# Linxyhaha/AtSpeed

Hardware: AMD Instinct MI355X
Metric: recommended items/sec (K=20 beams per user), mean accepted length alongside (higher is better)
Workload: dtype bf16; 1 GPU; Beauty V=32859, Llama-68M draft / Llama-7B(32L) target, K=20, DK=40, gamma=4, L=4, 256 user(s) per lock-step batch per GPU, position-set mask; users_per_gpu=1280, parallelism=user-shard x1

## Files before the change

### atspeed_amd/_lib.py

```python
from __future__ import annotations

import ctypes as C
import os
from typing import Optional

_HERE = os.path.dirname(os.path.abspath(__file__))
LIB_PATH = os.path.abspath(os.environ["ATSPEED_LIB"]) if os.environ.get("ATSPEED_LIB") else os.path.join(_HERE, "lib", "libatspeed_hip.so")

ATSPEED_F32, ATSPEED_BF16, ATSPEED_F16 = 0, 1, 2
WEIGHTS_ROW_MAJOR, WEIGHTS_PACKED = 0, 1
MAX_BEAMS, MAX_NEW_TOKENS, MAX_GAMMA = 64, 16, 8
LORA_MAX_RANK = 64
LORA_MAX_ADAPTERS = 16
ERR_INVALID, ERR_HIP, ERR_CAPACITY, ERR_CONSTRAINT, ERR_NO_DEVICE, ERR_FILTERED = -1, -2, -3, -4, -5, -6
EPI_STORE, EPI_F32, EPI_RESID, EPI_SWIGLU = 0, 1, 2, 3
MASK_BLOCK, MASK_ALLOW = 0, 1


class LlamaLayerWeights(C.Structure):
    _fields_ = [("input_norm", C.c_void_p), ("wqkv", C.c_void_p), ("wo", C.c_void_p),
                ("post_norm", C.c_void_p), ("wgu", C.c_void_p), ("wd", C.c_void_p)]


class LlamaConfig(C.Structure):
    _fields_ = [("vocab_size", C.c_int32), ("hidden", C.c_int32), ("n_layers", C.c_int32), ("n_heads", C.c_int32),
                ("ffn", C.c_int32), ("rope_theta", C.c_float), ("rms_eps", C.c_float), ("dtype", C.c_int32),
                ("max_slots", C.c_int32), ("max_tokens", C.c_int32), ("max_logit_rows", C.c_int32), ("weight_layout", C.c_int32)]


class LoraLayer(C.Structure):
    _fields_ = [("a_q", C.c_void_p), ("b_q", C.c_void_p), ("a_k", C.c_void_p), ("b_k", C.c_void_p), ("a_v", C.c_void_p), ("b_v", C.c_void_p)]


class LoraSlot(C.Structure):
    _fields_ = [("a_cat", C.c_void_p), ("b_q", C.c_void_p), ("b_k", C.c_void_p), ("b_v", C.c_void_p), ("r16", C.c_int32), ("scaling", C.c_float)]


class GenStats(C.Structure):
    _fields_ = [("n_run", C.c_int32), ("total_accept_steps", C.c_int32), ("accept_steps", C.c_int32 * MAX_NEW_TOKENS),
                ("n_valid", C.c_int32), ("n_target_forwards", C.c_int32), ("n_draft_forwards", C.c_int32),
                ("draft_ms", C.c_float), ("target_ms", C.c_float), ("verify_ms", C.c_float), ("total_ms", C.c_float),
                ("status", C.c_int32), ("n_target_passes", C.c_int32)]


class SessionCounters(C.Structure):
    _fields_ = [("rounds", C.c_int64), ("target_forwards", C.c_int64), ("draft_forwards", C.c_int64), ("lane_rounds", C.c_int64),
                ("users_admitted", C.c_int64), ("users_retired", C.c_int64), ("allocs_after_create", C.c_int64),
                ("arena_reserved", C.c_int32), ("arena_failed", C.c_int32), ("n_lanes", C.c_int32), ("lanes_occupied", C.c_int32),
                ("queued", C.c_int64), ("target_passes", C.c_int64)]


class SessionDone(C.Structure):
    _fields_ = [("ticket", C.c_int64), ("lane", C.c_int32), ("status", C.c_int32), ("rounds_queued", C.c_int64),
                ("rounds_in_lane", C.c_int64)]


class SessionUser(C.Structure):
    _fields_ = [("struct_size", C.c_size_t), ("prompt_ids_dev", C.c_void_p), ("prompt_len", C.c_int32), ("start_node", C.c_int32),
                ("seed", C.c_uint32), ("out_tokens_dev", C.c_void_p), ("out_scores_dev", C.c_void_p), ("stats_host", C.POINTER(GenStats)),
                ("masks", C.c_void_p), ("mask_user", C.c_int32), ("adapter", C.c_int32)]


_P, _I, _F, _SZ, _U32, _U64 = C.c_void_p, C.c_int32, C.c_float, C.c_size_t, C.c_uint32, C.c_uint64
_SEGS = [_I, _P, _P, _P, _P, _P, _P, _P, _P, _P]
SIGNATURES = {
    "atspeed_version": (C.c_char_p, []),
    "atspeed_last_error": (C.c_char_p, []),
    "atspeed_device_count": (C.c_int, []),
    "atspeed_fill_hash_normal": (C.c_int, [_P, _SZ, _U32, _F, _F, C.c_int, _U64, _P]),
    "atspeed_fsm_create": (C.c_int, [_P, _P, _P, _I, _I, _I, C.POINTER(_P)]),
    "atspeed_fsm_destroy": (None, [_P]),
    "atspeed_fsm_create_free": (C.c_int, [_I, C.POINTER(_P)]),
    "atspeed_fsm_set_id_filter": (C.c_int, [_P, _I, _I]),
    "atspeed_row_topk": (C.c_int, [_P, _I, _I, _I, _I, _P, _P]),
    "atspeed_beam_expand_prune_free": (C.c_int, [_P, _I, _P, _P, _I, _I, _I, _P, _P, _P, _P, _P, _P]),
    "atspeed_trie_flatten": (C.c_int, [_P, _P, _I, _P, _P, _P, C.POINTER(_I), C.POINTER(_I)]),
    "atspeed_llama_create": (C.c_int, [C.POINTER(LlamaConfig), _P, _P, _P, C.POINTER(LlamaLayerWeights), C.POINTER(_P)]),
    "atspeed_llama_destroy": (None, [_P]),
    "atspeed_llama_forward": (C.c_int, [_P, _P, _P, _P, _P, _I, _I, _I, _P, _P]),
    "atspeed_llama_forward_batch": (C.c_int, [_P, _I, _P, _P, _P, _P, _P, _P, _P, _P, _P]),
    "atspeed_llama_logits": (_P, [_P]),
    "atspeed_llama_read": (C.c_int, [_P, _I, _I, _P, _SZ, _P]),
    "atspeed_probe_mfma_bf16": (C.c_int, [_I, _P, C.c_size_t, _P, _P]),
    "atspeed_probe_hbm_read": (C.c_int, [_P, C.c_size_t, _I, _P, _P, _P]),
    "atspeed_llama_enable_fp8": (C.c_int, [_P, _P]),
    "atspeed_llama_fp8_counters": (C.c_int, [_P, _P, _P, _I]),
    "atspeed_llama_enable_fp4": (C.c_int, [_P, _P]),
    "atspeed_llama_fp4_counters": (C.c_int, [_P, _P, _P, _I]),
    "atspeed_quant_weights_mxfp4": (C.c_int, [_P, _I, _I, _I, _I, _P, _P, _P]),
    "atspeed_gemm_w4a8": (C.c_int, [_P, _P, _P, _P, _P, _I, _I, _I, _I, _I, _I, _I, _P, _SZ, _P]),
    "atspeed_llama_rope_fused_launches": (C.c_int64, [_P, _I]),
    "atspeed_llama_sk_arena_bytes": (C.c_int64, [_P]),
    "atspeed_llama_set_lora": (C.c_int, [_P, _I, _F, C.POINTER(LoraLayer), _P]),
    "atspeed_llama_clear_lora": (C.c_int, [_P]),
    "atspeed_llama_lora_launches": (C.c_int64, [_P, _I]),
# ... 184 lines not shown
```

### atspeed_amd/beamSD.py

```python
from __future__ import annotations

import ctypes as C
import time
import weakref
from types import SimpleNamespace
from typing import Dict, Optional

import numpy as np
import torch

from . import _lib
from .generation_trie import ConstraintFSM, SuffixTrieConstraint, WholeSentenceTrieConstraint, free_constraint
from .model import HipLlama


class Timer:

    def __init__(self, func="", sync_cuda=True, syn_device=0):
        self.func = func
        self.sync_cuda = sync_cuda
        self.syn_device = syn_device

    def _sync(self):
        if self.sync_cuda and torch.cuda.is_available():
# ... 364 lines not shown
    for i in range(n):
        o0, P = k * (int(off[i]) + i * L), int(off[i + 1] - off[i])
        res.append({"beam_sequence": out[o0: o0 + k * (P + L)].view(k, P + L), "beam_scores": scores[i]})
    return res


def _batch_call(entry, c: SimpleNamespace, k: int, max_new_tokens: int, *middle):
    n = len(c.prompts)
    ptrs, ints = C.c_void_p * n, C.c_int32 * n
    with torch.cuda.device(c.dev):
        ids32, toks, scores, keep = _batch_buffers(c.prompts, k, max_new_tokens, c.dev)
        stats = (_lib.GenStats * n)()
        try:
            _lib.check(entry(ptrs(*[d.handle for d in c.decs]), n, ptrs(*[t.data_ptr() for t in ids32]),
                             ints(*[int(p.numel()) for p in c.prompts]), c.dfsm.handle, ints(*[f.start for f in c.fsms]), *middle,
                             ptrs(*[t.data_ptr() for t in toks]), ptrs(*[t.data_ptr() for t in scores]), stats, _lib.stream_ptr(c.dev)))
        finally:
            if c.filter_owners:
                _clear_filters(c.decs)
    return (keep, toks, scores, k), stats


MAX_USERS_PER_CALL = 256


def _chunk_of(lists, i: int, n: int):
    return None if lists is None else lists[i:i + n]


def _chunked(call, inputs_list, mode):
    outs = []
    for i in range(0, len(inputs_list), MAX_USERS_PER_CALL):
        outs += call(inputs_list[i:i + MAX_USERS_PER_CALL], (mode[2] + i) if mode[0] else None, i)
    return outs


def _bssd_stats(st, k: int) -> Dict:
    n_run = int(st.n_run)
    total = int(st.total_accept_steps)
    return {
        "n_run": n_run,
        "total_accept_steps": total,
        "total_accept_tokens": total * k,
        "ave_accept_tokens": total * k / n_run if n_run else 0.0,
        "draft_time_cost": st.draft_ms * 1e-3,
        "target_time_cost": st.target_ms * 1e-3,
        "verify_time_cost": st.verify_ms * 1e-3,
        "device_time_cost": st.total_ms * 1e-3,
        "accept_steps": [int(st.accept_steps[i]) for i in range(min(n_run, _lib.MAX_NEW_TOKENS))],
        "n_valid": int(st.n_valid),
        "n_target_forwards": int(st.n_target_forwards),
        "n_draft_forwards": int(st.n_draft_forwards),
        "n_target_passes": int(st.n_target_passes),
    }


@Timer()
@torch.no_grad()
def BSSD(target_model, draft_model, inputs: Dict, gamma: int, max_new_tokens: int,
         logits_processor=None, prefix_allowed_tokens_fn=None, seed=None, trace_decisions: bool = False,
         exclude_items=None, allow_items=None, adapter=None) -> Dict:
    mode = _mode(seed, target_model, draft_model)
    filters = _filter_specs(1, exclude_items, allow_items, False, "BSSD")
    slots = _adapter_slots(target_model, adapter, 1, False, "BSSD")
    if _host_path(logits_processor, prefix_allowed_tokens_fn):
        _refuse_host_filters(filters, "BSSD")
        _refuse_host_adapters(slots, "BSSD")
        from .hostmask import bssd_host_mask
        return _host_call(bssd_host_mask, (target_model, draft_model), inputs, (int(gamma), int(max_new_tokens)), logits_processor,
                          prefix_allowed_tokens_fn, mode)
    k = int(target_model.generation_config.num_beams)
    dk = int(draft_model.generation_config.num_beams)
    c = _setup(target_model, draft_model, [inputs], prefix_allowed_tokens_fn, mode, "BSSD", trace_decisions, filters, adapters=slots)
    out, stats = _one_user_call(_lib.load().atspeed_bssd_generate, c, k, max_new_tokens, int(gamma), int(max_new_tokens), k, dk)
    out.update(_bssd_stats(stats, k))
    return out


beam_sd_generate = BSSD


class BSSDSession:

    def __init__(self, target_model, draft_model, lanes: int, gamma: int, max_new_tokens: int, prefix_allowed_tokens_fn=None,
                 max_prompt: Optional[int] = None, seed=None, logits_processor=None, trace_decisions: bool = False, _cached_decoders: bool = False):
        self.mode = _mode(seed, target_model, draft_model)
        if _host_path(logits_processor, prefix_allowed_tokens_fn):
            raise ValueError("BSSDSession runs on the device only: the mask must be able to compile() itself and there is no logits_processor")
        if trace_decisions:
            raise ValueError("BSSDSession keeps no decision trace: use BSSD / BSSD_batch with trace_decisions=True")
        if not 1 <= int(lanes) <= MAX_USERS_PER_CALL:
            raise ValueError(f"BSSDSession: lanes must be in 1 .. {MAX_USERS_PER_CALL}, not {lanes}")
        self.target, self.draft, self.fn = target_model, draft_model, prefix_allowed_tokens_fn
        self.n_lanes, self.gamma, self.max_new_tokens = int(lanes), int(gamma), int(max_new_tokens)
        self.k = int(target_model.generation_config.num_beams)
        self.dk = int(draft_model.generation_config.num_beams)
        self.max_prompt = int(max_prompt) if max_prompt is not None else min(target_model.max_tokens, 512)
        self.dev = target_model.device
        self._cached_decoders = _cached_decoders
        self._owner = self._decs = self._dfsm = self._fsm0 = None
        self._users: Dict[int, SimpleNamespace] = {}
        self._done_buf = (_lib.SessionDone * (2 * self.n_lanes))()
        self._submitted, self._closed = 0, False

    def _create(self, fsm: ConstraintFSM) -> None:
        lib = _lib.load()
# ... 271 lines not shown
```

### atspeed_amd/csrc/engine.hip

```cpp
#include <math.h>
#include <stdarg.h>
#include <string.h>

#include <algorithm>
#include <map>
#include <memory>
#include <mutex>
#include <vector>

#include "internal.h"
#include "session_queue.h"

static thread_local std::string g_last_error;

void atspeed_set_error(const char* fmt, ...) {
  char buf[1024];
  va_list ap;
  va_start(ap, fmt);
  vsnprintf(buf, sizeof(buf), fmt, ap);
  va_end(ap);
  g_last_error = buf;
}

extern "C" const char* atspeed_last_error(void) { return g_last_error.c_str(); }
std::atomic<long long> g_ats_lazy_allocs{0};
extern "C" const char* atspeed_version(void) { return "atspeed_hip 0.2 (gfx950)"; }

namespace {
constexpr int ATS_VERIFY_STAGED_TOKENS = 4096;
constexpr int ATS_VERIFY_STAGED_PASS_TOKENS = 1024;
constexpr int ATS_TAIL_ROWS_TOKENS = 512;
struct SwDef { const char* name; const char* env; int dflt; };
const SwDef kSwitches[ATS_N_SW] = {{"gemm_sk", "ATSPEED_GEMM_SK", 1},           {"gemm_sk_g", nullptr, 0},
                                   {"gemm_panel", "ATSPEED_GEMM_PANEL", 1},     {"gemm_force_mt", "ATSPEED_GEMM_FORCE_MT", 0},
                                   {"graphs", "ATSPEED_GRAPHS", 0},             {"fuse_qkv_rope", "ATSPEED_FUSE_QKV_ROPE", 1},
                                   {"gemm_kcut", "ATSPEED_GEMM_KCUT", 2},       {"fuse_qkv_reduce", "ATSPEED_FUSE_QKV_REDUCE", 1},
                                   {"verify_staged", "ATSPEED_VERIFY_STAGED", 1},
                                   {"verify_staged_tokens", "ATSPEED_VERIFY_STAGED_TOKENS", ATS_VERIFY_STAGED_TOKENS},
                                   {"verify_staged_pass_tokens", "ATSPEED_VERIFY_STAGED_PASS_TOKENS", ATS_VERIFY_STAGED_PASS_TOKENS},
                                   {"tail_rows_tokens", "ATSPEED_TAIL_ROWS_TOKENS", ATS_TAIL_ROWS_TOKENS},
                                   {"attn_short", "ATSPEED_ATTN_SHORT", 1}};
std::atomic<int> g_switch[ATS_N_SW];
std::once_flag g_switch_once;
void switches_init() {
  std::call_once(g_switch_once, [] {
    for (int i = 0; i < ATS_N_SW; ++i) {
      const char* v = kSwitches[i].env ? getenv(kSwitches[i].env) : nullptr;
      g_switch[i].store(v ? atoi(v) : kSwitches[i].dflt, std::memory_order_relaxed);
    }
  });
}
}
int ats_switch(int id) { switches_init(); return g_switch[id].load(std::memory_order_relaxed); }
extern "C" int atspeed_set_switch(const char* name, int32_t value) {
  ATS_REQUIRE(name, ATSPEED_ERR_INVALID, "set_switch: null name");
  switches_init();
  for (int i = 0; i < ATS_N_SW; ++i)
    if (!strcmp(name, kSwitches[i].name)) { g_switch[i].store(value, std::memory_order_relaxed); return ATSPEED_OK; }
  atspeed_set_error("set_switch: unknown switch '%s'", name);
  return ATSPEED_ERR_INVALID;
}
extern "C" int atspeed_get_switch(const char* name, int32_t* value_out) {
  ATS_REQUIRE(name && value_out, ATSPEED_ERR_INVALID, "get_switch: null argument");
  switches_init();
  for (int i = 0; i < ATS_N_SW; ++i)
    if (!strcmp(name, kSwitches[i].name)) { *value_out = g_switch[i].load(std::memory_order_relaxed); return ATSPEED_OK; }
  atspeed_set_error("get_switch: unknown switch '%s'", name);
  return ATSPEED_ERR_INVALID;
}
std::atomic<long long> g_ats_path_cnt[ATS_N_PATHS];
extern "C" int atspeed_gemm_path_counters(int64_t* out, int32_t n, int32_t reset) {
  for (int i = 0; i < ATS_N_PATHS; ++i) {
    const long long v = reset ? g_ats_path_cnt[i].exchange(0) : g_ats_path_cnt[i].load();
    if (out && i < n) out[i] = v;
  }
  return ATS_N_PATHS;
}
extern "C" int atspeed_device_count(void) {
  int n = 0;
  if (hipGetDeviceCount(&n) != hipSuccess) return 0;
  return n;
}

namespace {
struct StageRing {
  char *host = nullptr, *dev = nullptr;
  size_t cap = 0, used = 0;
};
thread_local StageRing g_stage_dev[ATS_MAX_DEVICES];
constexpr size_t kStageBytes = 8u << 20;
}

static int stage_slot(const void* host_obj, size_t bytes, hipStream_t st, StageRing** ring_out, size_t* off_out) {
  const int dev = ats_cur_device();
// ... 1348 lines not shown
struct RoundCtl {
  bool flat_trace;
  bool keep_filtered;
  bool lock_step;
  bool any = false;
  int target_forwards = 0, draft_forwards = 0;
  int target_passes = 0;
};

static bool bssd_round_staged(const std::vector<atspeed_decoder*>& ver, const std::vector<atspeed_decoder*>& fin) {
  const int mode = ats_switch(ATS_SW_VERIFY_STAGED);
  if (mode <= 0 || ver.empty()) return false;
  const atspeed_llama* T = ver[0]->target;
  if (!T->fp8.empty() || !T->fp4.empty() || T->has_lora()) return false;
  long long tok = 0;
  for (const atspeed_decoder* d : ver) { if (d->sample) return false; tok += d->run.n0 + d->run.dl * d->run.dk; }
  for (const atspeed_decoder* d : fin) { if (d->sample) return false; tok += d->run.n0; }
  if (mode >= 2) return true;
  if (tok <= ats_switch(ATS_SW_VERIFY_STAGED_TOKENS)) return false;
  const int pass_tok = ats_switch(ATS_SW_VERIFY_STAGED_PASS_TOKENS);
  if (pass_tok <= 0) return true;
  double skipped = 0., users_at[ATSPEED_MAX_GAMMA + 1] = {};
  for (const atspeed_decoder* d : ver)
    for (int j = 1; j <= d->run.dl; ++j) {
      const double q = T->stg_drafted[j] >= 1. ? T->stg_needed[j] / T->stg_drafted[j] : 0.;
      skipped += (1. - q) * d->run.dk;
      users_at[j] += q;
    }
  int extra = 0;
  for (int j = 1; j <= ATSPEED_MAX_GAMMA; ++j) extra += users_at[j] >= 0.5 ? 1 : 0;
  return skipped > (double)extra * pass_tok;
}

static int bssd_round(atspeed_decoder** decs, int n, hipStream_t st, hipEvent_t* g_ev, RoundCtl& ctl) {
  atspeed_llama *T = decs[0]->target, *D = decs[0]->draft;
  const int W = decs[0]->W;
  std::vector<atspeed_decoder*> ver, fin;
  int max_dl = 0;
  for (int u = 0; u < n; ++u) {
    atspeed_decoder* d = decs[u];
    atspeed_decoder::Run& r = d->run;
    if (r.done) continue;
    ATS_REQUIRE(T->slot_ok(d->adapter), ATSPEED_ERR_INVALID, "bssd: a user names adapter slot %d, which the target no longer holds", d->adapter);
    r.final_step = r.export_only = false;
    if (r.gen >= r.max_new) { r.final_step = r.export_only = true; continue; }
    r.dl = std::min(r.gamma, r.max_new - r.gen - 1);
    if (r.dl == 0) { r.final_step = true; fin.push_back(d); continue; }
    ATS_REQUIRE(r.n0 + r.dl * r.dk <= d->tok_cap, ATSPEED_ERR_CAPACITY, "bssd: packed target input too long");
    ATS_REQUIRE(r.base + r.n0 + r.dl * r.dk <= T->cfg.max_slots, ATSPEED_ERR_CAPACITY,
                "bssd: KV slots exhausted (%d needed, %d available)", r.base + r.n0 + r.dl * r.dk, T->cfg.max_slots);
    ver.push_back(d);
    max_dl = std::max(max_dl, r.dl);
  }
  hipEventRecord(g_ev[0], st);
  for (int i = 0; i < max_dl; ++i) {
    SegTable t{};
    std::vector<BeamStepArgs> args;
    std::vector<WarpCutArgs> wargs;
    std::vector<atspeed_decoder*> us;
    for (atspeed_decoder* d : ver) if (d->run.dl > i) us.push_back(d);
    for (atspeed_decoder* d : us) {
      atspeed_decoder::Run& r = d->run;
      TokBuf& tin = d->tin[r.cur];
      Seg sg;
      if (i == 0) sg = r.reingest ? make_seg(d->dround, r.dk + r.k, r.base + r.n0, r.nb, d->dkv)
                                  : make_seg(tin, r.n0, r.base + r.n0, r.nb, d->dkv);
      else        sg = make_seg(tb_offset(tin, r.n0 + (i - 1) * r.dk, W), r.dk, r.base + r.n0 + i * r.dk, r.dk, d->dkv);
      t.seg[t.n++] = sg;
      r.s.n_draft_forwards++;
    }
    ATS_TRY(ats_seg_finish(t));
    ATS_TRY(decode_forward(D, t, decs[0]->run.fsm, decs[0]->run.dk, st));
    ctl.draft_forwards++;
    for (size_t j = 0; j < us.size(); ++j) {
      atspeed_decoder* d = us[j];
      atspeed_decoder::Run& r = d->run;
      BeamStepArgs a = beam_step_args(d, D, t.seg[j], r.fsm, i == 0 ? d->round_beams[r.cur] : d->blk[i], d->blk[i + 1], r.gen + i, r.dk);
      beam_step_emit(a, d->tin[r.cur], i == 0 ? r.n0 - r.nb : r.n0 + (i - 1) * r.dk, r.n0 + i * r.dk, r.base + r.n0 + i * r.dk);
      if (a.sample) {
        a.rng_sub = ats_rng_sub(d->seed, ATS_RNG_STEP, r.s.n_run, i, 1);
        a.tab_score = d->tab_score + (size_t)i * ATS_MAX_CAND; a.tab_off = d->tab_off + (size_t)i * (MAXB + 1); a.tab_lse = d->tab_lse + i;
      }
      if (a.cutoff) wargs.push_back(warp_cut_args(d, a));
      args.push_back(a);
    }
    ATS_TRY(warp_cutoffs(wargs, st));
    const BeamStepArgs* dev_args = nullptr;
    ATS_TRY(stage_args(args, &dev_args, st));
    ATS_TRY(ats_beam_step_multi(dev_args, (int)args.size(), st));
  }
  hipEventRecord(g_ev[1], st);
  hipEventRecord(g_ev[5], st);
  float ms_t = 0.f, ms_v = 0.f;
  if (!ver.empty() || !fin.empty()) {
    const bool staged = ctl.lock_step && bssd_round_staged(ver, fin);
    std::vector<VerifyArgs> vall(ver.size());
    std::vector<size_t> pend(ver.size());
    for (size_t j = 0; j < ver.size(); ++j) pend[j] = j;
    int row_off = 0;
    for (int p = 0;; ++p) {
      SegTable t{};
      for (size_t j : pend) {
        atspeed_decoder* d = ver[j];
        atspeed_decoder::Run& r = d->run;
        const int Tn = r.n0 + r.dl * r.dk;
        if (!staged)     t.seg[t.n++] = make_seg(d->tin[r.cur], Tn, r.base + Tn, r.nb + r.dl * r.dk, d->tkv, d->adapter);
        else if (p == 0) t.seg[t.n++] = make_seg(d->tin[r.cur], r.n0, r.base + r.n0, r.nb, d->tkv, d->adapter);
        else             t.seg[t.n++] = make_seg(tb_offset(d->tin[r.cur], r.n0 + (p - 1) * r.dk, W), r.dk, r.base + r.n0 + p * r.dk, r.dk, d->tkv, d->adapter);
        if (p == 0) r.s.n_target_forwards++;
        r.s.n_target_passes++;
      }
      if (p == 0) for (atspeed_decoder* d : fin) {
        atspeed_decoder::Run& r = d->run;
        t.seg[t.n++] = make_seg(d->tin[r.cur], r.n0, r.base + r.n0, r.nb, d->tkv, d->adapter);
        r.s.n_target_forwards++; r.s.n_target_passes++;
      }
      ATS_TRY(ats_seg_finish(t));
      ATS_TRY(decode_forward(T, t, decs[0]->run.fsm, decs[0]->run.k, st, row_off));
      if (p == 0) ctl.target_forwards++;
      ctl.target_passes++;
      hipEventRecord(g_ev[2], st);
      std::vector<VerifyArgs> vargs;
      std::vector<WarpCutArgs> wargs;
      const ActCtx* cx = T->act;
      for (size_t i = 0; i < pend.size(); ++i) {
        atspeed_decoder* d = ver[pend[i]];
        atspeed_decoder::Run& r = d->run;
        VerifyArgs& va = vall[pend[i]];
        if (p == 0) {
          va.blk[0] = d->round_beams[r.cur];
          for (int b = 1; b <= r.dl; ++b) va.blk[b] = d->blk[b];
          va.nb = r.nb; va.dl = r.dl; va.k = r.k; va.dk = r.dk; va.gen_len0 = r.gen;
          va.ld = T->logits_ld; va.fsm = d->fsm_dev(r.fsm); va.n_row_cand = r.k;
          va.cur = d->tin[r.cur]; va.n0 = r.n0; va.next = d->tin[r.cur ^ 1]; va.dnext = d->dround; va.vis_words = W;
          va.res = d->round_beams[r.cur ^ 1]; va.mail = d->mail_dev;
          va.vtrace = (d->trace_level >= 1 && !d->sample) ? d->vtrace_dev : nullptr;
          if (d->sample) {
            va.sample = 1; va.temperature = d->temperature; va.seed = d->seed; va.round = r.s.n_run;
            for (int b = 0; b < r.dl; ++b) {
              va.dtab_score[b] = d->tab_score + (size_t)b * ATS_MAX_CAND; va.dtab_off[b] = d->tab_off + (size_t)b * (MAXB + 1);
              va.dtab_lse[b] = d->tab_lse + b;
            }
          }
        }
        if (!staged) {
          const RowViews rv = seg_rows(T, t.seg[i]);
          va.logits = rv.logits; va.lse = rv.lse; va.row_cand = rv.row_cand;
          for (int b = 1; b <= r.dl; ++b) va.blk_row0[b] = r.nb + (b - 1) * r.dk;
          va.blocks_ready = r.dl + 1;
        } else {
          va.logits = cx->logits; va.lse = cx->lse; va.row_cand = cx->row_cand;
          va.blk_row0[p] = row_off + t.seg[i].logit_row0;
          va.blocks_ready = p + 1;
        }
        if (d->warps()) { va.cutoff = d->cutoff; wargs.push_back(warp_cut_args(d, va)); }
        vargs.push_back(va);
      }
      std::vector<BeamStepArgs> fargs;
      if (p == 0) for (size_t j = 0; j < fin.size(); ++j) {
        atspeed_decoder* d = fin[j];
        atspeed_decoder::Run& r = d->run;
        BeamStepArgs a = beam_step_args(d, T, t.seg[ver.size() + j], r.fsm, d->round_beams[r.cur], d->round_beams[r.cur ^ 1], r.gen, r.k);
        if (a.sample) a.rng_sub = ats_rng_sub(d->seed, ATS_RNG_STEP, r.s.n_run, 0, 0);
        if (a.cutoff) wargs.push_back(warp_cut_args(d, a));
        fargs.push_back(a);
      }
      ATS_TRY(warp_cutoffs(wargs, st));
      if (!vargs.empty()) {
        const VerifyArgs* dv = nullptr;
        ATS_TRY(stage_args(vargs, &dv, st));
        ATS_TRY(ats_verify_walk_multi(dv, (int)vargs.size(), st));
      }
      if (!fargs.empty()) {
        const BeamStepArgs* df = nullptr;
        ATS_TRY(stage_args(fargs, &df, st));
        ATS_TRY(ats_beam_step_multi(df, (int)fargs.size(), st));
      }
      if (p == 0) for (atspeed_decoder* d : fin) { d->run.cur ^= 1; d->run.gen += 1; }
      bool more = false;
      for (size_t j : pend) more = more || (staged && ver[j]->run.dl > p);
      if (!more) break;
      hipEventRecord(g_ev[3], st);
      ATS_HIP(hipStreamSynchronize(st));
      ats_stage_reset();
      float a_ms = 0.f, b_ms = 0.f;
      hipEventElapsedTime(&a_ms, g_ev[1], g_ev[2]);
      hipEventElapsedTime(&b_ms, g_ev[2], g_ev[3]);
      ms_t += a_ms; ms_v += b_ms;
      std::vector<size_t> next;
      for (size_t j : pend) if (ver[j]->mail_host->n_matches == ATS_WALK_PENDING && ver[j]->mail_host->status == 0) next.push_back(j);
      row_off += t.total_logit;
      pend.swap(next);
      hipEventRecord(g_ev[1], st);
      hipEventRecord(g_ev[2], st);
      if (pend.empty()) break;
    }
  } else {
    hipEventRecord(g_ev[2], st);
  }
  hipEventRecord(g_ev[3], st);
  std::vector<ExportBeamsArgs> ex;
  for (int u = 0; u < n; ++u) {
    atspeed_decoder* d = decs[u];
    atspeed_decoder::Run& r = d->run;
    if (!r.done && r.final_step) ex.push_back(ExportBeamsArgs{d->round_beams[r.cur], r.out_tokens, r.out_scores, d->sample ? 1 : 0});
  }
  if (!ex.empty()) ATS_TRY(export_beams(ex, decs[0]->run.k, decs[0]->run.max_new, st));
  for (int u = 0; u < n; ++u) {
    atspeed_decoder* d = decs[u];
    atspeed_decoder::Run& r = d->run;
    if (r.done) continue;
    if (r.final_step) {}
    else if (ctl.flat_trace)
      for (int i = 1; i <= r.dl; ++i)
        ATS_HIP(hipMemcpyAsync(d->trace_host + (i - 1) * MAXB, d->blk[i].flat, sizeof(int32_t) * r.dk, hipMemcpyDeviceToHost, st));
    if (d->trace_level >= 1 && !r.export_only)
      ATS_HIP(hipMemcpyAsync(d->dump_host, d->beam_area, d->beam_area_bytes, hipMemcpyDeviceToHost, st));
  }
  ATS_HIP(hipStreamSynchronize(st));
  ats_stage_reset();
  float ms_d = 0.f, ms_tl = 0.f, ms_vl = 0.f;
  hipEventElapsedTime(&ms_d, g_ev[0], g_ev[5]);
  hipEventElapsedTime(&ms_tl, g_ev[1], g_ev[2]);
  hipEventElapsedTime(&ms_vl, g_ev[2], g_ev[3]);
  ms_t += ms_tl; ms_v += ms_vl;
  int n_act = 0;
  for (int u = 0; u < n; ++u) if (!decs[u]->run.done) ++n_act;
  if (!ver.empty() && !ver[0]->sample)
    for (int j = 1; j <= ATSPEED_MAX_GAMMA; ++j) { T->stg_drafted[j] *= 0.5; T->stg_needed[j] *= 0.5; }
  ctl.any = false;
  for (int u = 0; u < n; ++u) {
    atspeed_decoder* d = decs[u];
    atspeed_decoder::Run& r = d->run;
    if (r.done) continue;
    if (ctl.keep_filtered && d->mail_host->status == ATSPEED_ERR_FILTERED) {
      r.s.n_valid = 0; r.s.status = ATSPEED_ERR_FILTERED;
      ATS_TRY(blank_outputs(r.out_tokens, r.out_scores, r.k, r.max_new, st));
      r.s.total_ms = r.s.draft_ms + r.s.target_ms + r.s.verify_ms;
      if (r.stats_out) *r.stats_out = r.s;
      r.done = true;
      continue;
    }
    ATS_TRY(mailbox_status(d));
    r.s.draft_ms += ms_d / n_act; r.s.target_ms += ms_t / n_act; r.s.verify_ms += ms_v / n_act;
    if (r.final_step) {
      if (d->trace_level >= 1 && !r.export_only) decisions_append(d, 1, r.nb, 0, 0, r.gen - 1, r.k, r.dk, {r.cur ^ 1, r.cur});
      r.s.n_valid = d->mail_host->n_valid;
      r.s.total_ms = r.s.draft_ms + r.s.target_ms + r.s.verify_ms;
      if (r.stats_out) *r.stats_out = r.s;
      r.done = true;
      continue;
    }
    const int nm = d->mail_host->n_matches, dl = r.dl, dk = r.dk;
    ATS_REQUIRE(nm >= 0 && nm <= dl, ATSPEED_ERR_HIP, "bssd: a verify walk reported %d accepted steps of %d", nm, dl);
    if (!d->sample) for (int j = 1; j <= dl; ++j) { T->stg_drafted[j] += 1.; T->stg_needed[j] += nm >= j ? 1. : 0.; }
    if (ctl.flat_trace) {
      d->trace.push_back(dl); d->trace.push_back(nm); d->trace.push_back(r.nb);
      for (int i = 0; i < dl; ++i) for (int j = 0; j < dk; ++j) d->trace.push_back(d->trace_host[i * MAXB + j]);
    }
    if (d->trace_level >= 1) {
      std::vector<int> blocks{r.cur};
      for (int i = 1; i <= dl; ++i) blocks.push_back(2 + i);
      blocks.push_back(r.cur ^ 1);
      decisions_append(d, 0, r.nb, dl, nm, r.gen, r.k, dk, blocks);
    }
    if (r.s.n_run < ATSPEED_MAX_NEW_TOKENS) r.s.accept_steps[r.s.n_run] = nm;
    r.s.n_run++;
    r.s.total_accept_steps += nm;
    r.base += r.n0 + nm * dk;
    r.n0 = r.k; r.nb = r.k;
    r.gen += nm + 1;
    r.reingest = (nm == dl);
    r.cur ^= 1;
    ctl.any = true;
  }
  return ATSPEED_OK;
}

// ... 346 lines not shown
```

### atspeed_amd/csrc/internal.h

```cpp
#pragma once
#include <atomic>

#include "common.h"

constexpr int ATS_MAX_SEGS = 256;
constexpr int ATS_MAX_QTILES = ATS_MAX_SEGS * 8;
struct Seg {
  const int32_t* ids; const int32_t* pos; const int32_t* slot; const uint64_t* vis;
  void* kc; void* vc;
  int row0, n_tok;
  int n_slots;
  int logit_row0, n_logit;
  int adapter;
};
struct SegTable {
  int n, total_tok, total_logit;
  int n_qtiles;
  int qtile_rows;
  Seg seg[ATS_MAX_SEGS];
  unsigned char qtile_seg[ATS_MAX_QTILES], qtile_idx[ATS_MAX_QTILES];
};
#if defined(__HIPCC__)
__device__ __forceinline__ int seg_of_row(const SegTable* t, int row) {
  int lo = 0, hi = t->n;
  while (hi - lo > 1) { int mid = (lo + hi) >> 1; if (t->seg[mid].row0 <= row) lo = mid; else hi = mid; }
  return lo;
}
#endif
struct RowInfo { void* kc; void* vc; int pos; int slot; };
static_assert(sizeof(RowInfo) == 24, "RowInfo is part of the C ABI (atspeed_segs_row_info) and one 24-byte load in the qkv epilogues");
int ats_seg_finish(SegTable& t, int qtile_rows = 0);
struct RopeEpi { const RowInfo* rows = nullptr; const float* cos_tab = nullptr; const float* sin_tab = nullptr; size_t layer_off = 0; int hidden = 0; };
int ats_stage(const void* host_obj, size_t bytes, const void** dev_out, hipStream_t st);
int ats_stage_to(const void* host_obj, size_t bytes, void* dev_dst, hipStream_t st);
void ats_stage_reset();

struct SkArena { float* ws = nullptr; int* cnt = nullptr; };
constexpr size_t ATS_SK_ARENA_BYTES = (size_t)512 * 256 * 1024;
constexpr int ATS_SK_ARENA_COUNTERS = 256;

enum { ATS_PATH_RING = 0, ATS_PATH_RING_SK = 1, ATS_PATH_WDMA = 2, ATS_PATH_WDMA_SPLIT = 3, ATS_PATH_RING_SPLIT = 4, ATS_PATH_TILED = 5,
       ATS_PATH_FP8_RING = 6, ATS_PATH_FP8_WDMA = 7, ATS_PATH_FP8_WDMA_SPLIT = 8, ATS_PATH_PANEL = 9, ATS_PATH_PANEL_SPLIT = 10, ATS_PATH_FP8_RING_SPLIT = 11,
       ATS_PATH_FP4 = 12 ,
       ATS_PATH_ATTN32_1BUF = 13, ATS_PATH_ATTN32_2BUF = 14 ,
       ATS_N_PATHS = 16 };
extern std::atomic<long long> g_ats_path_cnt[ATS_N_PATHS];
extern std::atomic<long long> g_ats_lazy_allocs;
inline void ats_count_path(int p) { g_ats_path_cnt[p].fetch_add(1, std::memory_order_relaxed); }

enum { ATS_SW_GEMM_SK = 0,
       ATS_SW_GEMM_SK_G,
       ATS_SW_GEMM_PANEL,
       ATS_SW_GEMM_FORCE_MT,
       ATS_SW_GRAPHS,
       ATS_SW_FUSE_QKV_ROPE,
       ATS_SW_GEMM_KCUT,
       ATS_SW_FUSE_QKV_REDUCE,
       ATS_SW_VERIFY_STAGED,
       ATS_SW_VERIFY_STAGED_TOKENS,
       ATS_SW_VERIFY_STAGED_PASS_TOKENS,
       ATS_SW_TAIL_ROWS_TOKENS,
       ATS_SW_ATTN_SHORT,
       ATS_N_SW };
int ats_switch(int id);

enum { EPI_STORE = 0, EPI_F32 = 1, EPI_RESID = 2, EPI_SWIGLU = 3, EPI_F32_LSE = 4 ,
       EPI_QKV_ROPE = 5  };
namespace ats_bf16 {
#include "kernels_decl.inc"
}
namespace ats_f16 {
#include "kernels_decl.inc"
}

struct FsmDev {
  const int32_t* row_ptr;
  const int32_t* tok;
  const int32_t* nxt;
  int32_t n_nodes, n_edges, vocab;
  int32_t filter_min, filter_eos;
  const uint32_t* blocked;
};
struct atspeed_fsm {
  FsmDev dev;
  int32_t *d_row_ptr, *d_tok, *d_nxt;
  unsigned char* d_tile_store;
};

struct atspeed_node_masks {
  const atspeed_fsm* fsm;
  int n_users, words;
  uint32_t* bits;
  void* block;
};
struct NodeMaskBuild {
  FsmDev fsm;
  const int32_t* start;  const int32_t* seq_tok;  const int32_t* seq_off;  const int32_t* user_off;
  int32_t* path;
  int32_t* len;
  uint32_t* bits;  uint32_t* kept;  uint32_t* ends;
  int32_t* unknown;  int32_t* status;
  int words, mode;
};
int ats_node_masks_build(const NodeMaskBuild& b, int n_users, hipStream_t st);
inline const uint32_t* ats_mask_bits(const atspeed_node_masks* m, int user) { return m ? m->bits + (size_t)user * m->words : nullptr; }

struct TokBuf {
  int32_t* ids;
  int32_t* pos;
  int32_t* slot;
  uint64_t* vis;
};
struct BeamSet {
  float* score;
  int32_t* node;
// ... 79 lines not shown
```

### include/atspeed_hip.h

```cpp
#ifndef ATSPEED_HIP_H
#define ATSPEED_HIP_H

#include <stddef.h>
#include <stdint.h>

#ifdef __cplusplus
extern "C" {
#endif

typedef enum atspeed_status {
  ATSPEED_OK = 0,
  ATSPEED_ERR_INVALID = -1,
  ATSPEED_ERR_HIP = -2,
  ATSPEED_ERR_CAPACITY = -3,
  ATSPEED_ERR_CONSTRAINT = -4,
  ATSPEED_ERR_NO_DEVICE = -5,
  ATSPEED_ERR_FILTERED = -6
} atspeed_status;

typedef enum atspeed_dtype { ATSPEED_F32 = 0, ATSPEED_BF16 = 1, ATSPEED_F16 = 2 } atspeed_dtype;

#define ATSPEED_MAX_BEAMS 64
#define ATSPEED_MAX_NEW_TOKENS 16
#define ATSPEED_MAX_GAMMA 8
// ... 80 lines not shown
int atspeed_llama_forward_batch_adapters(atspeed_llama* m, int32_t n, const int32_t* const* ids_dev, const int32_t* const* pos_dev,
                                         const int32_t* const* slots_dev, const uint64_t* const* vis_bits_dev, const int32_t* n_tokens,
                                         const int32_t* n_slots_visible, const int32_t* n_logit_rows, const int32_t* adapters ,
                                         float* logits_out_dev, void* stream);

int atspeed_lmhead_lse(const void* x_dev, const void* w_dev, float* logits_dev, float* lse_dev, int32_t rows, int32_t vocab,
                       int32_t hidden, int32_t ld, const atspeed_fsm* fsm , void* workspace_dev, size_t workspace_bytes,
                       int32_t* fused_out , void* stream);

int atspeed_lse_rows(const float* logits_dev, int32_t n_rows, int32_t vocab, int32_t ld,
                     float* lse_out_dev, void* stream);

int atspeed_log_softmax_rows(const float* logits_dev, int32_t ld, const float* lse_dev, int32_t n_rows, int32_t vocab, float* out_dev,
                             int32_t ld_out, void* stream);

int atspeed_beam_expand_prune(const float* logits_dev, int32_t ld, const float* lse_dev,
                              const float* beam_score_dev, const int32_t* beam_node_dev, int32_t n_rows,
                              const atspeed_fsm* fsm, int32_t k,
                              float* out_score_dev, int32_t* out_parent_dev, int32_t* out_token_dev,
                              int32_t* out_node_dev, int32_t* out_flat_dev, void* stream);

int atspeed_row_topk(const float* scores_dev, int32_t n_rows, int32_t vocab, int32_t ld, int32_t k, int32_t* out_tokens_dev, void* stream);
int atspeed_beam_expand_prune_free(const float* logits_dev, int32_t ld, const float* lse_dev, const float* beam_score_dev, int32_t n_rows,
                                   int32_t vocab, int32_t k, int32_t* row_cand_ws_dev, float* out_score_dev, int32_t* out_parent_dev,
                                   int32_t* out_token_dev, int32_t* out_flat_dev, void* stream);

int atspeed_accept(const int32_t* target_flat_dev, const float* target_score_dev, int32_t k,
                   const int32_t* draft_flat_dev, int32_t dk,
                   int32_t* hit_out_dev, float* score_by_hit_out_dev, int32_t* accept_out_dev, void* stream);

typedef struct atspeed_decoder atspeed_decoder;
int atspeed_decoder_create(atspeed_llama* target, atspeed_llama* draft ,
                           int32_t max_prompt, atspeed_decoder** out);
void atspeed_decoder_destroy(atspeed_decoder* d);

int atspeed_decoder_set_sampling(atspeed_decoder* d, int32_t do_sample, float temperature, uint32_t seed);

int atspeed_decoder_set_warpers(atspeed_decoder* d, int32_t top_k, float top_p, int32_t min_tokens_to_keep);

int atspeed_warp_cutoffs(const float* logits_dev, int32_t ld, const float* lse_dev, int32_t n_rows, const atspeed_fsm* fsm,
                         const int32_t* nodes_dev, float temperature, int32_t top_k, float top_p, int32_t min_tokens_to_keep,
                         float* cutoffs_out_dev, void* stream);
int64_t atspeed_warp_cutoff_launches(void);

typedef struct atspeed_gen_stats {
  int32_t n_run;
  int32_t total_accept_steps;
  int32_t accept_steps[ATSPEED_MAX_NEW_TOKENS];
  int32_t n_valid;
  int32_t n_target_forwards, n_draft_forwards;
  float draft_ms, target_ms, verify_ms, total_ms;
  int32_t status;
  int32_t n_target_passes;
} atspeed_gen_stats;

int atspeed_bssd_generate(atspeed_decoder* d, const int32_t* prompt_ids_dev, int32_t prompt_len,
                          const atspeed_fsm* fsm, int32_t start_node, int32_t gamma, int32_t max_new_tokens,
                          int32_t k, int32_t dk, int32_t* out_tokens_dev, float* out_scores_dev,
                          atspeed_gen_stats* stats_host, void* stream);

int atspeed_bssd_generate_batch(atspeed_decoder** decoders, int32_t n, const int32_t* const* prompt_ids_dev,
                                const int32_t* prompt_lens, const atspeed_fsm* fsm, const int32_t* start_nodes,
                                int32_t gamma, int32_t max_new_tokens, int32_t k, int32_t dk,
                                int32_t* const* out_tokens_dev, float* const* out_scores_dev,
                                atspeed_gen_stats* stats_host , void* stream);

typedef struct atspeed_session atspeed_session;
typedef struct atspeed_session_counters {
  int64_t rounds;
  int64_t target_forwards;
  int64_t draft_forwards;
  int64_t lane_rounds;
  int64_t users_admitted, users_retired;
  int64_t allocs_after_create;
  int32_t arena_reserved;
  int32_t arena_failed;
  int32_t n_lanes, lanes_occupied;
  int64_t queued;
  int64_t target_passes;
} atspeed_session_counters;
int atspeed_session_create(atspeed_decoder* const* lanes, int32_t n_lanes, const atspeed_fsm* fsm, int32_t gamma, int32_t max_new_tokens,
                           int32_t k, int32_t dk, int32_t max_prompt, void* stream, atspeed_session** out);
int atspeed_session_submit(atspeed_session* s, const int32_t* prompt_ids_dev, int32_t prompt_len, int32_t start_node, uint32_t seed,
                           int32_t* out_tokens_dev, float* out_scores_dev, atspeed_gen_stats* stats_host, int64_t* ticket_out);
typedef struct atspeed_session_done {
  int64_t ticket;
  int32_t lane, status;
  int64_t rounds_queued;
  int64_t rounds_in_lane;
} atspeed_session_done;
int atspeed_session_round(atspeed_session* s, atspeed_session_done* done_out, int32_t cap, int32_t* n_out);
int atspeed_session_drain(atspeed_session* s, atspeed_session_done* done_out, int32_t cap, int32_t* n_out);
int atspeed_session_get_counters(const atspeed_session* s, atspeed_session_counters* out);
void atspeed_session_destroy(atspeed_session* s);

typedef struct atspeed_node_masks atspeed_node_masks;
#define ATSPEED_MASK_BLOCK 0
#define ATSPEED_MASK_ALLOW 1
int atspeed_node_masks_create(const atspeed_fsm* fsm, int32_t n_users, const int32_t* start_nodes, const int32_t* seq_tokens,
                              const int32_t* seq_offsets, const int32_t* user_seq_offsets, int32_t mode, int32_t* unknown_out ,
                              int32_t* status_out , void* stream, atspeed_node_masks** out);
void atspeed_node_masks_destroy(atspeed_node_masks* masks);
int atspeed_node_masks_read(const atspeed_node_masks* masks, int32_t user, uint32_t* words_out_host, int32_t n_words);
int atspeed_decoder_set_node_mask(atspeed_decoder* d, const atspeed_node_masks* masks, int32_t user);
int atspeed_session_submit_masked(atspeed_session* s, const int32_t* prompt_ids_dev, int32_t prompt_len, int32_t start_node, uint32_t seed,
                                  int32_t* out_tokens_dev, float* out_scores_dev, atspeed_gen_stats* stats_host,
// ... 109 lines not shown
```

Measured before the change: 12230 items/s.

## Draft speculative steps lazily, interleaved with staged verification passes

When staged lock-step verification is active, only the first draft step runs upfront. Each later draft step runs inside the verify pass loop and only for users whose verification is still pending. Drafting for users whose earlier tokens were already rejected is skipped, saving draft forwards and beam-step work. In exchange, draft and verify now serialise per pass, adding launch and sync overhead. A new n_draft_passes stat and a switch (default on) are added.

```diff
diff --git a/atspeed_amd/_lib.py b/atspeed_amd/_lib.py
--- a/atspeed_amd/_lib.py
+++ b/atspeed_amd/_lib.py
@@ -40,7 +40,7 @@
     _fields_ = [("n_run", C.c_int32), ("total_accept_steps", C.c_int32), ("accept_steps", C.c_int32 * MAX_NEW_TOKENS),
                 ("n_valid", C.c_int32), ("n_target_forwards", C.c_int32), ("n_draft_forwards", C.c_int32),
                 ("draft_ms", C.c_float), ("target_ms", C.c_float), ("verify_ms", C.c_float), ("total_ms", C.c_float),
-                ("status", C.c_int32), ("n_target_passes", C.c_int32)]
+                ("status", C.c_int32), ("n_target_passes", C.c_int32), ("n_draft_passes", C.c_int32)]
 
 
 class SessionCounters(C.Structure):
diff --git a/atspeed_amd/beamSD.py b/atspeed_amd/beamSD.py
--- a/atspeed_amd/beamSD.py
+++ b/atspeed_amd/beamSD.py
@@ -440,6 +440,7 @@
         "n_target_forwards": int(st.n_target_forwards),
         "n_draft_forwards": int(st.n_draft_forwards),
         "n_target_passes": int(st.n_target_passes),
+        "n_draft_passes": int(st.n_draft_passes),
     }
 
 
diff --git a/atspeed_amd/csrc/engine.hip b/atspeed_amd/csrc/engine.hip
--- a/atspeed_amd/csrc/engine.hip
+++ b/atspeed_amd/csrc/engine.hip
@@ -39,7 +39,8 @@
                                    {"verify_staged_tokens", "ATSPEED_VERIFY_STAGED_TOKENS", ATS_VERIFY_STAGED_TOKENS},
                                    {"verify_staged_pass_tokens", "ATSPEED_VERIFY_STAGED_PASS_TOKENS", ATS_VERIFY_STAGED_PASS_TOKENS},
                                    {"tail_rows_tokens", "ATSPEED_TAIL_ROWS_TOKENS", ATS_TAIL_ROWS_TOKENS},
-                                   {"attn_short", "ATSPEED_ATTN_SHORT", 1}};
+                                   {"attn_short", "ATSPEED_ATTN_SHORT", 1},
+                                   {"draft_lazy", "ATSPEED_DRAFT_LAZY", 1}};
 std::atomic<int> g_switch[ATS_N_SW];
 std::once_flag g_switch_once;
 void switches_init() {
@@ -1494,13 +1495,16 @@
     ver.push_back(d);
     max_dl = std::max(max_dl, r.dl);
   }
-  hipEventRecord(g_ev[0], st);
-  for (int i = 0; i < max_dl; ++i) {
+  const bool staged = ctl.lock_step && bssd_round_staged(ver, fin);
+  bool lazy = staged && ats_switch(ATS_SW_DRAFT_LAZY) > 0 && !ctl.flat_trace;
+  for (atspeed_decoder* d : ver) {
+    lazy = lazy && d->trace_level < 1;
+    d->run.s.n_draft_forwards += d->run.dl;
+  }
+  auto draft_step = [&](int i, const std::vector<atspeed_decoder*>& us) -> int {
     SegTable t{};
     std::vector<BeamStepArgs> args;
     std::vector<WarpCutArgs> wargs;
-    std::vector<atspeed_decoder*> us;
-    for (atspeed_decoder* d : ver) if (d->run.dl > i) us.push_back(d);
     for (atspeed_decoder* d : us) {
       atspeed_decoder::Run& r = d->run;
       TokBuf& tin = d->tin[r.cur];
@@ -1509,7 +1513,7 @@
                                   : make_seg(tin, r.n0, r.base + r.n0, r.nb, d->dkv);
       else        sg = make_seg(tb_offset(tin, r.n0 + (i - 1) * r.dk, W), r.dk, r.base + r.n0 + i * r.dk, r.dk, d->dkv);
       t.seg[t.n++] = sg;
-      r.s.n_draft_forwards++;
+      r.s.n_draft_passes++;
     }
     ATS_TRY(ats_seg_finish(t));
     ATS_TRY(decode_forward(D, t, decs[0]->run.fsm, decs[0]->run.dk, st));
@@ -1529,18 +1533,35 @@
     ATS_TRY(warp_cutoffs(wargs, st));
     const BeamStepArgs* dev_args = nullptr;
     ATS_TRY(stage_args(args, &dev_args, st));
-    ATS_TRY(ats_beam_step_multi(dev_args, (int)args.size(), st));
+    return ats_beam_step_multi(dev_args, (int)args.size(), st);
+  };
+  hipEventRecord(g_ev[0], st);
+  for (int i = 0; i < (lazy ? std::min(max_dl, 1) : max_dl); ++i) {
+    std::vector<atspeed_decoder*> us;
+    for (atspeed_decoder* d : ver) if (d->run.dl > i) us.push_back(d);
+    ATS_TRY(draft_step(i, us));
   }
   hipEventRecord(g_ev[1], st);
   hipEventRecord(g_ev[5], st);
-  float ms_t = 0.f, ms_v = 0.f;
+  float ms_t = 0.f, ms_v = 0.f, ms_dl = 0.f;
+  bool lazy_open = false;
   if (!ver.empty() || !fin.empty()) {
-    const bool staged = ctl.lock_step && bssd_round_staged(ver, fin);
     std::vector<VerifyArgs> vall(ver.size());
     std::vector<size_t> pend(ver.size());
     for (size_t j = 0; j < ver.size(); ++j) pend[j] = j;
     int row_off = 0;
     for (int p = 0;; ++p) {
+      if (lazy && p >= 1) {
+        std::vector<atspeed_decoder*> us;
+        for (size_t j : pend) if (ver[j]->run.dl > p) us.push_back(ver[j]);
+        if (!us.empty()) {
+          hipEventRecord(g_ev[6], st);
+          ATS_TRY(draft_step(p, us));
+          hipEventRecord(g_ev[7], st);
+          hipEventRecord(g_ev[1], st);
+          lazy_open = true;
+        }
+      }
       SegTable t{};
       for (size_t j : pend) {
         atspeed_decoder* d = ver[j];
@@ -1629,6 +1650,7 @@
       hipEventElapsedTime(&a_ms, g_ev[1], g_ev[2]);
       hipEventElapsedTime(&b_ms, g_ev[2], g_ev[3]);
       ms_t += a_ms; ms_v += b_ms;
+      if (lazy_open) { float d_ms = 0.f; hipEventElapsedTime(&d_ms, g_ev[6], g_ev[7]); ms_dl += d_ms; lazy_open = false; }
       std::vector<size_t> next;
       for (size_t j : pend) if (ver[j]->mail_host->n_matches == ATS_WALK_PENDING && ver[j]->mail_host->status == 0) next.push_back(j);
       row_off += t.total_logit;
@@ -1666,6 +1688,8 @@
   hipEventElapsedTime(&ms_tl, g_ev[1], g_ev[2]);
   hipEventElapsedTime(&ms_vl, g_ev[2], g_ev[3]);
   ms_t += ms_tl; ms_v += ms_vl;
+  if (lazy_open) { float d_ms = 0.f; hipEventElapsedTime(&d_ms, g_ev[6], g_ev[7]); ms_dl += d_ms; }
+  ms_d += ms_dl;
   int n_act = 0;
   for (int u = 0; u < n; ++u) if (!decs[u]->run.done) ++n_act;
   if (!ver.empty() && !ver[0]->sample)
diff --git a/atspeed_amd/csrc/internal.h b/atspeed_amd/csrc/internal.h
--- a/atspeed_amd/csrc/internal.h
+++ b/atspeed_amd/csrc/internal.h
@@ -61,6 +61,7 @@
        ATS_SW_VERIFY_STAGED_PASS_TOKENS,
        ATS_SW_TAIL_ROWS_TOKENS,
        ATS_SW_ATTN_SHORT,
+       ATS_SW_DRAFT_LAZY,
        ATS_N_SW };
 int ats_switch(int id);
 
diff --git a/include/atspeed_hip.h b/include/atspeed_hip.h
--- a/include/atspeed_hip.h
+++ b/include/atspeed_hip.h
@@ -156,6 +156,7 @@
   float draft_ms, target_ms, verify_ms, total_ms;
   int32_t status;
   int32_t n_target_passes;
+  int32_t n_draft_passes;
 } atspeed_gen_stats;
 
 int atspeed_bssd_generate(atspeed_decoder* d, const int32_t* prompt_ids_dev, int32_t prompt_len,
```

Measured after the change: 12350 items/s, median of 6. No clear change (+1.0%).
